# YuxiaWu/RAG4DyG

Measured on AMD Instinct MI355X. Metric: query-seqs/sec encode+top-k over full pool, higher is better.
Workload: dtype f32 (f16x2 operands: two fp16 terms, three products, f32 accumulate)

## Files before the change

include/r4d.h:

```cpp
#ifndef R4D_H
#define R4D_H

#include <stddef.h>
#include <stdint.h>

#ifdef __cplusplus
extern "C" {
#endif

#define R4D_OK 0
#define R4D_ERR_INVALID (-1)
#define R4D_ERR_HIP (-2)
#define R4D_ERR_WORKSPACE (-3)

#define R4D_ABI_VERSION 6

int r4d_abi_version(void);
int r4d_build_flags(void);
const char* r4d_last_error(void);

typedef struct r4d_gpt2_config {
    int32_t n_layer;
    int32_t n_head;
    int32_t n_embd;
// ... 80 lines not shown

int r4d_lm_logits_f32(const float* hidden_d, const float* wte_d, int32_t M, int32_t V, int32_t d,
                      float* logits_d, void* stream);

int r4d_set_attention_fused(int32_t mode);

int r4d_set_attention_h2(int32_t on);
int r4d_set_attention_kblk(int32_t on);
int r4d_pack_kblk_words(const uint32_t* qkv_words_d, int64_t rows, int32_t n_head, int32_t d, uint32_t* kblk_d, void* stream);
int r4d_attention_h2_kblk_f32(const uint32_t* qkv_words_d, const uint32_t* kblk_d, int32_t B, int32_t T, int32_t n_head, int32_t d,
                              float* a_d, void* stream);
int r4d_pack_h2_words_f32(const float* x_d, int64_t n, uint32_t* words_d, void* stream);
int r4d_attention_h2_f32(const uint32_t* qkv_words_d, int32_t B, int32_t T, int32_t n_head, int32_t d, float* a_d, void* stream);

int r4d_set_gemm_h2p(int32_t on);
int r4d_layernorm_lines_f32(const float* x_d, const float* w_d, const float* b_d, int32_t rows, int32_t d, float eps,
                            uint16_t* y_lines_d, void* stream);
int r4d_split2_lines_f16(const float* x_d, int64_t rows, int32_t K, uint16_t* lines_d, void* stream);
int r4d_conv1d_h2p_f32(const uint16_t* x_lines_d, const uint16_t* planes_d, const float* bias_d, const float* residual_d, int32_t M,
                       int32_t K, int32_t N, int32_t epilogue, int32_t out_lines, void* y_d, void* stream);

#define R4D_RANGE_NONFINITE_HIDDEN 1u
#define R4D_RANGE_BAD_NORM 2u
#define R4D_RANGE_BAD_LABEL 4u
int r4d_set_range_flag(uint32_t* flag_d);

int r4d_layernorm_f32(const float* x_d, const float* w_d, const float* b_d, int32_t rows, int32_t d,
                      float eps, float* y_d, void* stream);
int r4d_conv1d_f32(const float* x_d, const float* w_d, const float* w_t_d ,
                   const float* bias_d, const float* residual_d,
// ... 150 lines not shown
```

rag4dyg_amd/_lib.py:

```python
import ctypes
import os
from ctypes import POINTER, Structure, c_char_p, c_double, c_float, c_int32, c_int64, c_size_t, c_uint32, c_uint64, c_void_p

PKG = os.path.dirname(os.path.abspath(__file__))
LIB_PATH = os.environ.get("R4D_LIB_PATH") or os.path.join(PKG, "librag4dyg_hip.so")

R4D_ABI_VERSION = 6
HEAD_GRAD_UNTIED, HEAD_GRAD_TIED, HEAD_GRAD_NONE = 0, 1, 2


class R4DError(RuntimeError):
    pass


class GPT2ConfigC(Structure):
    _fields_ = [("n_layer", c_int32), ("n_head", c_int32), ("n_embd", c_int32), ("vocab", c_int32),
                ("n_positions", c_int32), ("ln_eps", c_float)]


class GPT2LayerC(Structure):
    _fields_ = [(n, c_void_p) for n in ("ln_1_w", "ln_1_b", "c_attn_w", "c_attn_b", "attn_proj_w", "attn_proj_b",
                                         "ln_2_w", "ln_2_b", "c_fc_w", "c_fc_b", "mlp_proj_w", "mlp_proj_b",
                                         "c_attn_wT", "attn_proj_wT", "c_fc_wT", "mlp_proj_wT",
                                         "c_attn_w3", "attn_proj_w3", "c_fc_w3", "mlp_proj_w3",
# ... 38 lines not shown
    "r4d_gpt2_workspace_bytes": (c_size_t, [POINTER(GPT2ConfigC), c_int32, c_int32]),
    "r4d_gpt2_encode_f32": (c_int32, [POINTER(GPT2ConfigC), POINTER(GPT2WeightsC), _P, _P, c_int32, c_int32,
                                      _P, _P, _P, _P, _P, c_size_t, _P]),
    "r4d_gpt2_groups_workspace_bytes": (c_size_t, [POINTER(GPT2ConfigC), c_int32, POINTER(c_int32), POINTER(c_int32)]),
    "r4d_gpt2_encode_groups_f32": (c_int32, [POINTER(GPT2ConfigC), POINTER(GPT2WeightsC), c_int32, POINTER(_P),
                                             POINTER(c_int32), POINTER(c_int32), _P, _P, c_size_t, _P]),
    "r4d_gpt2_encode_groups_ex_f32": (c_int32, [POINTER(GPT2ConfigC), POINTER(GPT2WeightsC), c_int32, POINTER(_P), POINTER(_P),
                                                POINTER(c_int32), POINTER(c_int32), _P, _P, _P, _P, c_size_t, _P]),
    "r4d_set_attention_fused": (c_int32, [c_int32]),
    "r4d_set_attention_h2": (c_int32, [c_int32]),
    "r4d_set_attention_kblk": (c_int32, [c_int32]),
    "r4d_pack_kblk_words": (c_int32, [_P, c_int64, c_int32, c_int32, _P, _P]),
    "r4d_attention_h2_kblk_f32": (c_int32, [_P, _P, c_int32, c_int32, c_int32, c_int32, _P, _P]),
    "r4d_set_range_flag": (c_int32, [_P]),
    "r4d_set_gemm_h2p": (c_int32, [c_int32]),
    "r4d_layernorm_lines_f32": (c_int32, [_P, _P, _P, c_int32, c_int32, c_float, _P, _P]),
    "r4d_split2_lines_f16": (c_int32, [_P, c_int64, c_int32, _P, _P]),
    "r4d_conv1d_h2p_f32": (c_int32, [_P, _P, _P, _P, c_int32, c_int32, c_int32, c_int32, c_int32, _P, _P]),
    "r4d_pack_h2_words_f32": (c_int32, [_P, c_int64, _P, _P]),
    "r4d_attention_h2_f32": (c_int32, [_P, c_int32, c_int32, c_int32, c_int32, _P, _P]),
    "r4d_gpt2_decode_workspace_bytes": (c_size_t, [POINTER(GPT2ConfigC), c_int32]),
    "r4d_gpt2_decode_step_f32": (c_int32, [POINTER(GPT2ConfigC), POINTER(GPT2WeightsC), _P, _P, _P, _P, c_int32, c_int32,
                                           _P, _P, c_size_t, _P]),
    "r4d_gpt2_greedy_workspace_bytes": (c_size_t, [POINTER(GPT2ConfigC), c_int32]),
    "r4d_gpt2_greedy_step_f32": (c_int32, [POINTER(GPT2ConfigC), POINTER(GPT2WeightsC), POINTER(GreedyStateC), _P, c_int32,
                                           c_int32, _P, c_size_t, _P]),
    "r4d_gpt2_greedy_graph_create": (c_int32, [POINTER(GPT2ConfigC), POINTER(GPT2WeightsC), POINTER(GreedyStateC), _P,
                                               c_int32, c_int32, _P, c_size_t, POINTER(_P)]),
    "r4d_decode_graph_launch": (c_int32, [_P, c_int32, _P]),
    "r4d_decode_graph_destroy": (None, [_P]),
# ... 105 lines not shown
```

rag4dyg_amd/csrc/common.h:

```cpp
#pragma once
#include <hip/hip_runtime.h>
#include <stdint.h>
#include <stdio.h>
#include <stdarg.h>
#include "../../include/r4d.h"

namespace r4d {

void set_error(const char* fmt, ...);
int dbgflag_kc(); int dbgflag_att(); int dbgflag_sk(); int dbgflag_jac(); int dbgflag_scan(); int dbgflag_s3(); int dbgflag_h2();

#define R4D_REQUIRE(cond, ...)                     \
    do {                                           \
        if (!(cond)) {                             \
            r4d::set_error(__VA_ARGS__);           \
            return R4D_ERR_INVALID;                \
        }                                          \
    } while (0)

#define R4D_HIP(call)                                                                  \
    do {                                                                               \
        hipError_t e_ = (call);                                                        \
        if (e_ != hipSuccess) {                                                        \
            r4d::set_error("%s: %s", #call, hipGetErrorString(e_));                    \
// ... 101 lines not shown
struct S3Args {
    const float* A; const unsigned short* planes; float* C;
    const float* bias; const float* resid;
    int M, N, K, lda, ldc, ldr, epilogue;
    unsigned* kblk; int kb_hd;
};
bool gemm_s3_supported(int M, int K, int N);
int launch_gemm_s3(const S3Args& a, hipStream_t stream);
bool gemm_s3_f32b_supported(int M, int K, int N);
int launch_gemm_s3_f32b(const float* A, const float* B, float* C, int M, int N, int K, int lda, int ldc, int epilogue, hipStream_t stream);
int launch_gemm_s3_scan_order(const float* q_hat, const float* pool_hat, float* scores, int Q, int N, int d, int ng, hipStream_t stream);
bool gemm_h2_supported(int M, int K, int N);
int launch_gemm_h2(const S3Args& a, hipStream_t stream);
int launch_split2_planes(const float* w, int N, int K, long long ld_k, long long ld_n, unsigned short* planes, hipStream_t s);
extern int g_gemm_h2p;
bool gemm_h2p_supported(int M, int K, int N);
int launch_gemm_h2p(const S3Args& a, const unsigned short* a_lines, bool out_lines, hipStream_t stream);
int launch_split2_lines(const float* x, long long rows, int K, unsigned short* lines, hipStream_t s);
extern int g_gemm_split3;
int conv1d(const float* x, const float* w, const float* wT, const float* bias, const float* resid, int M, int K, int N,
           int epilogue, float* y, hipStream_t s, float* skinny_scratch = nullptr, bool sk_counters_zeroed = false,
           const unsigned short* w3 = nullptr, const unsigned short* w2h = nullptr);
bool gemm_s3tn_supported(int I, int J, int M, int lda, int ldb);
int gemm_s3tn_slices(int I, int J, int M, int max_slices);
int launch_gemm_s3tn(const float* X, const float* dY, float* out, int I, int J, int M, int lda, int ldb, int S, int* slices_out,
                     hipStream_t stream, float* db_partials = nullptr);
int launch_split3_planes(const float* w, int N, int K, long long ld_k, long long ld_n, unsigned short* planes, hipStream_t s);

struct DropKey { unsigned seed_lo, seed_hi, step_lo, step_hi; };
int launch_dropout(const float* x, const float* resid, long long n, float* out, float p, DropKey key, unsigned site,
// ... 90 lines not shown
```

rag4dyg_amd/csrc/gemm_h2p.hip:

```cpp
#include <stdlib.h>
#include <string.h>
#include "common.h"
#include "h2.h"

namespace r4d {

typedef float f32x16p __attribute__((ext_vector_type(16)));
typedef float f32x2p __attribute__((ext_vector_type(2)));
typedef unsigned int u32x4p __attribute__((ext_vector_type(4)));
typedef _Float16 f16x8p __attribute__((ext_vector_type(8)));

int g_gemm_h2p = 1;

__device__ __forceinline__ f32x2p gelu_new_h2p(f32x2p x) {
    const float k0 = -2.0f * 0.7978845608028654f * 1.4426950408889634f, k1 = 0.044715f * k0;
    const f32x2p a = x * x * k1 + k0;
    const f32x2p w = x * a;
    f32x2p e;
    e.x = __builtin_amdgcn_exp2f(w.x); e.y = __builtin_amdgcn_exp2f(w.y);
    e = e + 1.0f;
    f32x2p r;
    r.x = __builtin_amdgcn_rcpf(e.x); r.y = __builtin_amdgcn_rcpf(e.y);
    return x * r;
}
__device__ __forceinline__ float gelu_new_h2p_1(float x) {
    const float k0 = -2.0f * 0.7978845608028654f * 1.4426950408889634f, k1 = 0.044715f * k0;
    return x * __builtin_amdgcn_rcpf(1.0f + __builtin_amdgcn_exp2f(x * __builtin_fmaf(x * x, k1, k0)));
// ... 19 lines not shown
                 "global_load_lds_dwordx4 %2, %5 offset:1024\n\t"
                 "global_load_lds_dwordx4 %3, %5 offset:2048\n\t"
                 "global_load_lds_dwordx4 %4, %5 offset:3072\n\t"
                 "s_mov_b32 m0, %0"
                 : "=&s"(keep) : "v"(v0), "v"(v1), "v"(v2), "v"(v3), "s"(base), "s"(lds_dst) : "memory");
}
template <int N_> __device__ __forceinline__ void h2p_wait_vm() { asm volatile("s_waitcnt vmcnt(%0)" :: "n"(N_) : "memory"); }

template <int BM, int BN, int EPI, bool OUT_LINES, int WGM = 2, int WGN = 4>
__global__ __launch_bounds__(64 * WGM * WGN, (WGM * WGN) / 4) void gemm_h2p_kernel(const unsigned short* __restrict__ Al, const unsigned short* __restrict__ Bp,
                                                          float* __restrict__ Cg, const float* __restrict__ biasg,
                                                          const float* __restrict__ residg, const H2PShape g) {
    constexpr int NW = WGM * WGN;
    constexpr int WM = BM / WGM, WN = BN / WGN, TM = WM / 32, TN = WN / 32;
    constexpr int STAGE = (BM + BN) * 8;
    constexpr int NBUF = 3;
    constexpr int NGA = BM / 8 / NW, NGB = BN / 8 / NW;
    constexpr int NDMA = NGA + NGB;
    static_assert(BM == 128 && (BN == 256 || BN == 128) && TM >= 1 && TN >= 1 && (NGA == 2 || NGA == 4) && (NGB == 2 || NGB == 4 || NGB == 8), "tile");
    __shared__ u32x4p lds[NBUF * STAGE];

    const int nblk = gridDim.x, xq = nblk >> 3, xr = nblk & 7, xcd = blockIdx.x & 7;
    const int bid = xcd * xq + min(xcd, xr) + (blockIdx.x >> 3);
    constexpr int GROUP_M = 8;
    const int tiles_m = (g.M + BM - 1) / BM, tiles_n = (g.N + BN - 1) / BN;
    const int per_group = GROUP_M * tiles_n;
    const int grp = bid / per_group, first_m = grp * GROUP_M;
    const int gsz = min(tiles_m - first_m, GROUP_M);
    const int tile_m = first_m + (bid % per_group) % gsz, tile_n = (bid % per_group) / gsz;
    const int m0 = tile_m * BM, n0 = tile_n * BN;
    const int nkt = g.K / 32;

    const int tid = threadIdx.x, lane = tid & 63, wid = tid >> 6;
    const int wm = wid / WGN, wn = wid % WGN;
    const int li = lane & 31, lh = lane >> 5;

    unsigned va[NGA], vb[NGB];
    const int lrow = lane >> 3, lslot = lane & 7;
#pragma unroll
    for (int i = 0; i < NGA; ++i) {
        const int r = (wid * NGA + i) * 8 + lrow;
        va[i] = (unsigned)min(m0 + r, g.M - 1) * (unsigned)(g.K * 4) + 16u * (unsigned)(lslot ^ ((r >> 1) & 7)) + 3072u - 1024u * (i & 3);
    }
#pragma unroll
    for (int i = 0; i < NGB; ++i) {
        const int r = (wid * NGB + i) * 8 + lrow;
        vb[i] = (unsigned)min(n0 + r, g.N - 1) * (unsigned)(g.K * 4) + 16u * (unsigned)(lslot ^ ((r >> 1) & 7)) + 3072u - 1024u * (i & 3);
    }
    const unsigned lds0 = __builtin_amdgcn_readfirstlane((unsigned)(size_t)lds);
    const unsigned wid_s = __builtin_amdgcn_readfirstlane((unsigned)wid);
    const unsigned dst_a = lds0 + (wid_s * NGA) * 1024u, dst_b = lds0 + ((unsigned)(BM / 8) + wid_s * NGB) * 1024u;
    const char* abase = reinterpret_cast<const char*>(Al) - 3072;
    const char* bbase = reinterpret_cast<const char*>(Bp) - 3072;
#define H2P_ISSUE(KT, STG)                                                                         \
    {                                                                                              \
        const unsigned so_ = (unsigned)(STG) * (unsigned)(STAGE * 16);                             \
        if constexpr (NGA == 4) h2p_dma4(abase + (size_t)(KT) * 128, va[0], va[1], va[2], va[3], dst_a + so_); \
        else h2p_dma2(abase + (size_t)(KT) * 128, va[0], va[1], dst_a + so_);                      \
        if constexpr (NGB == 8) {                                                                  \
            h2p_dma4(bbase + (size_t)(KT) * 128, vb[0], vb[1], vb[2], vb[3], dst_b + so_);          \
            h2p_dma4(bbase + (size_t)(KT) * 128, vb[4], vb[5], vb[6], vb[7], dst_b + so_ + 4096u);   \
        } else if constexpr (NGB == 4) h2p_dma4(bbase + (size_t)(KT) * 128, vb[0], vb[1], vb[2], vb[3], dst_b + so_); \
        else h2p_dma2(bbase + (size_t)(KT) * 128, vb[0], vb[1], dst_b + so_);                       \
    }

    const int fsw = (li >> 1) & 7;
    int f_off[2][2];
#pragma unroll
    for (int s_ = 0; s_ < 2; ++s_)
#pragma unroll
        for (int p = 0; p < 2; ++p) f_off[s_][p] = li * 8 + ((4 * p + 2 * s_ + lh) ^ fsw);
    const int fa_base = wm * WM * 8, fb_base = BM * 8 + wn * WN * 8;

    f32x16p acc0[TM][TN], acc1[TM][TN];
#pragma unroll
    for (int i = 0; i < TM; ++i)
#pragma unroll
        for (int j = 0; j < TN; ++j)
#pragma unroll
            for (int r = 0; r < 16; ++r) { acc0[i][j][r] = 0.f; acc1[i][j][r] = 0.f; }

#define H2P_MFMA(ACC, A_, B_, I_, J_) \
    ACC[I_][J_] = __builtin_amdgcn_mfma_f32_32x32x16_f16(__builtin_bit_cast(f16x8p, A_), __builtin_bit_cast(f16x8p, B_), ACC[I_][J_], 0, 0, 0);
    u32x4p fa[2][TM][2], fb[2][TN][2];
#define H2P_FRAGS(SET, STG, S)                                                                     \
    {                                                                                              \
        const u32x4p* st_ = lds + (STG) * STAGE;                                                   \
                                        \
        _Pragma("unroll") for (int i = 0; i < TM; ++i) fa[SET][i][1] = st_[fa_base + i * 256 + f_off[S][1]]; \
        _Pragma("unroll") for (int j = 0; j < TN; ++j) fb[SET][j][0] = st_[fb_base + j * 256 + f_off[S][0]]; \
        _Pragma("unroll") for (int i = 0; i < TM; ++i) fa[SET][i][0] = st_[fa_base + i * 256 + f_off[S][0]]; \
        _Pragma("unroll") for (int j = 0; j < TN; ++j) fb[SET][j][1] = st_[fb_base + j * 256 + f_off[S][1]]; \
    }
#define H2P_MFMAS(SET)                                                                             \
    {                                                                                              \
        _Pragma("unroll") for (int i = 0; i < TM; ++i) _Pragma("unroll") for (int j = 0; j < TN; ++j) H2P_MFMA(acc1, fa[SET][i][1], fb[SET][j][0], i, j) \
        _Pragma("unroll") for (int i = 0; i < TM; ++i) _Pragma("unroll") for (int j = 0; j < TN; ++j) H2P_MFMA(acc0, fa[SET][i][0], fb[SET][j][0], i, j) \
        _Pragma("unroll") for (int i = 0; i < TM; ++i) _Pragma("unroll") for (int j = 0; j < TN; ++j) H2P_MFMA(acc1, fa[SET][i][0], fb[SET][j][1], i, j) \
    }

    H2P_ISSUE(0, 0)
    if (nkt > 1) { H2P_ISSUE(1, 1) h2p_wait_vm<NDMA>(); } else { h2p_wait_vm<0>(); }
    __syncthreads();
    H2P_FRAGS(0, 0, 0)

    constexpr int NMF = 3 * TM * TN, NFR = 2 * (TM + TN);
    static_assert(NMF >= NFR, "interleave");
#define H2P_ITER(CUR, NXT, WR)                                                                     \
    {                                                                                              \
        __builtin_amdgcn_sched_barrier(0);                                                         \
        const bool more_ = kt + 2 < nkt;                                                           \
        if (more_) H2P_ISSUE(kt + 2, WR)                                                           \
        H2P_FRAGS(1, CUR, 1)                                                                       \
        H2P_MFMAS(0)                                                                               \
        _Pragma("unroll") for (int m_ = 0; m_ < NMF; ++m_) {                                       \
            __builtin_amdgcn_sched_group_barrier(0x008, 1, 0);                                     \
            if (m_ < NFR) __builtin_amdgcn_sched_group_barrier(0x100, 1, 0);                       \
        }                                                                                          \
        __builtin_amdgcn_sched_barrier(0);                                                         \
        if (more_) h2p_wait_vm<NDMA>(); else h2p_wait_vm<0>();                                     \
        asm volatile("s_waitcnt lgkmcnt(0)\n\ts_barrier" ::: "memory");                            \
        H2P_FRAGS(0, NXT, 0)                                                                       \
        H2P_MFMAS(1)                                                                               \
        _Pragma("unroll") for (int m_ = 0; m_ < NMF; ++m_) {                                       \
            __builtin_amdgcn_sched_group_barrier(0x008, 1, 0);                                     \
            if (m_ < NFR) __builtin_amdgcn_sched_group_barrier(0x100, 1, 0);                       \
        }                                                                                          \
        __builtin_amdgcn_sched_barrier(0);                                                         \
    }
    int kt = 0;
    for (; kt + 2 < nkt; kt += 3) {
        H2P_ITER(0, 1, 2)
        { ++kt; H2P_ITER(1, 2, 0) }
        { ++kt; H2P_ITER(2, 0, 1) }
        kt -= 2;
    }
    if (kt < nkt) {
        H2P_ITER(0, 1, 2)
        if (kt + 1 < nkt) { ++kt; H2P_ITER(1, 2, 0) }
    }
#undef H2P_ITER
#undef H2P_FRAGS
#undef H2P_MFMAS
#undef H2P_MFMA
#undef H2P_ISSUE

    constexpr float UNS = H2_A_UNSCALE;
    float* __restrict__ C = Cg;
    const bool interior = (m0 + BM <= g.M) & (n0 + BN <= g.N);
    if constexpr (OUT_LINES) {
        static_assert(EPI == EPI_GELU, "line output: the c_fc epilogue only");
        unsigned char* __restrict__ L = reinterpret_cast<unsigned char*>(Cg);
        const long long row_bytes = (long long)g.N * 4;
        const bool odd = li & 1;
#pragma unroll
        for (int j = 0; j < TN; ++j) {
            const int colb = n0 + wn * WN + j * 32;
            const bool col_ok = colb + li < g.N;
            const float bias = (biasg && col_ok) ? biasg[colb + li] : 0.f;
#pragma unroll
            for (int i = 0; i < TM; ++i) {
#pragma unroll
                for (int r2 = 0; r2 < 16; r2 += 2) {
                    f32x2p v2 = {__builtin_fmaf(acc1[i][j][r2], H2_LO_UNSCALE, acc0[i][j][r2]) * UNS + bias,
                                 __builtin_fmaf(acc1[i][j][r2 + 1], H2_LO_UNSCALE, acc0[i][j][r2 + 1]) * UNS + bias};
                    v2 = gelu_new_h2p(v2);
                    const float vx = v2.x, vy = v2.y;
                    const float send = odd ? vx : vy;
                    const float recv = __builtin_bit_cast(float, __builtin_amdgcn_mov_dpp(__builtin_bit_cast(int, send), 0xB1, 0xF, 0xF, true));
                    const float c0 = odd ? recv : vx, c1 = odd ? vy : recv;
                    unsigned h, l;
                    split2_pair<true>(c0, c1, h, l);
                    const int r = r2 + (odd ? 1 : 0);
                    const int row = m0 + wm * WM + i * 32 + (r & 3) + 8 * (r >> 2) + 4 * lh;
                    if (interior || (row < g.M && col_ok)) {
                        unsigned* dst = reinterpret_cast<unsigned*>(L + (long long)row * row_bytes + (long long)(colb >> 5) * 128 + (li >> 1) * 4);
                        dst[0] = h;
                        dst[16] = l;
                    }
                }
            }
        }
        return;
    } else {
        if (interior) {
            const int lane_c = ((wm * WM + 4 * lh) * g.ldc + wn * WN + li) * 4;
            const int lane_r = ((wm * WM + 4 * lh) * g.ldr + wn * WN + li) * 4;
            const __amdgpu_buffer_rsrc_t c_rsrc = __builtin_amdgcn_make_buffer_rsrc(
                C + (long long)m0 * g.ldc + n0, 0, ((BM - 1) * g.ldc + BN) * 4, 0x00020000);
            const __amdgpu_buffer_rsrc_t r_rsrc = __builtin_amdgcn_make_buffer_rsrc(
                const_cast<float*>(EPI == EPI_RESIDUAL ? residg + (long long)m0 * g.ldr + n0 : Cg), 0,
                EPI == EPI_RESIDUAL ? ((BM - 1) * g.ldr + BN) * 4 : 0, 0x00020000);
            const int kd = g.N / 3;
            const __amdgpu_buffer_rsrc_t kb_rsrc = __builtin_amdgcn_make_buffer_rsrc(
                (EPI == EPI_H2WORDS && g.kb_hd) ? g.kblk : reinterpret_cast<unsigned*>(Cg), 0,
                (EPI == EPI_H2WORDS && g.kb_hd) ? ((g.M + 31) / 32) * (kd * 128) : 0, 0x00020000);
            const int lane_kb = (li >> 3) * 1024 + ((li >> 2) & 1) * 512 + ((li & 3) + 4 * lh) * 16;
#pragma unroll
            for (int j = 0; j < TN; ++j) {
                const float bias = biasg ? biasg[n0 + wn * WN + j * 32 + li] : 0.f;
                const int colb = n0 + wn * WN + j * 32;
                const bool to_kb = EPI == EPI_H2WORDS && g.kb_hd && colb >= kd && colb < 2 * kd;
                const int kb_chunk = to_kb ? ((colb - kd) / g.kb_hd) * (g.kb_hd / 8) + ((colb - kd) % g.kb_hd) / 8 : 0;
#pragma unroll
                for (int i = 0; i < TM; ++i) {
                    const int kb_soff = (((m0 + wm * WM + i * 32) >> 5) * (kd / 8) + kb_chunk) * 1024;
                    float res[16];
                    if (EPI == EPI_RESIDUAL) {
#pragma unroll
                        for (int r = 0; r < 16; ++r)
                            res[r] = __builtin_bit_cast(float, __builtin_amdgcn_raw_buffer_load_b32(
                                r_rsrc, lane_r, ((i * 32 + (r & 3) + 8 * (r >> 2)) * g.ldr + j * 32) * 4, 0));
                    }
                    unsigned o[16];
#pragma unroll
                    for (int r2 = 0; r2 < 16; r2 += 2) {
                        f32x2p v2 = {__builtin_fmaf(acc1[i][j][r2], H2_LO_UNSCALE, acc0[i][j][r2]) * UNS + bias,
                                     __builtin_fmaf(acc1[i][j][r2 + 1], H2_LO_UNSCALE, acc0[i][j][r2 + 1]) * UNS + bias};
                        if (EPI == EPI_GELU) v2 = gelu_new_h2p(v2);
                        else if (EPI == EPI_RESIDUAL) { v2.x += res[r2]; v2.y += res[r2 + 1]; }
                        const float vx = v2.x, vy = v2.y;
                        o[r2] = __builtin_bit_cast(unsigned int, vx); o[r2 + 1] = __builtin_bit_cast(unsigned int, vy);
                        if (EPI == EPI_H2WORDS) h2_words<true>(v2.x, v2.y, o[r2], o[r2 + 1]);
                    }
                    if (EPI == EPI_H2WORDS && to_kb) {
                        const bool o1 = li & 1, o2 = li & 2;
#pragma unroll
                        for (int a4 = 0; a4 < 16; a4 += 4) {
                            unsigned x0 = o[a4], x1 = o[a4 + 1], x2 = o[a4 + 2], x3 = o[a4 + 3];
                            {
                                const unsigned s01 = o1 ? x0 : x1, s23 = o1 ? x2 : x3;
                                const unsigned r01 = (unsigned)__builtin_amdgcn_mov_dpp((int)s01, 0xB1, 0xF, 0xF, true);
                                const unsigned r23 = (unsigned)__builtin_amdgcn_mov_dpp((int)s23, 0xB1, 0xF, 0xF, true);
                                if (o1) { x0 = r01; x2 = r23; } else { x1 = r01; x3 = r23; }
                            }
                            {
                                const unsigned s02 = o2 ? x0 : x2, s13 = o2 ? x1 : x3;
                                const unsigned r02 = (unsigned)__builtin_amdgcn_mov_dpp((int)s02, 0x4E, 0xF, 0xF, true);
                                const unsigned r13 = (unsigned)__builtin_amdgcn_mov_dpp((int)s13, 0x4E, 0xF, 0xF, true);
                                if (o2) { x0 = r02; x1 = r13; } else { x2 = r02; x3 = r13; }
                            }
                            const u32x4p slot = {x0, x1, x2, x3};
                            __builtin_amdgcn_raw_buffer_store_b128(slot, kb_rsrc, lane_kb, kb_soff + 2 * a4 * 16, 0);
                        }
                    } else {
#pragma unroll
                        for (int r = 0; r < 16; ++r)
                            __builtin_amdgcn_raw_buffer_store_b32(o[r], c_rsrc, lane_c, ((i * 32 + (r & 3) + 8 * (r >> 2)) * g.ldc + j * 32) * 4, 0);
                    }
                }
            }
            return;
        }
#pragma unroll
        for (int j = 0; j < TN; ++j) {
            const int col = n0 + wn * WN + j * 32 + li;
            const bool col_ok = col < g.N;
            const int colc = min(col, g.N - 1);
            const float bias = biasg ? biasg[colc] : 0.f;
#pragma unroll
            for (int i = 0; i < TM; ++i) {
#pragma unroll
                for (int r = 0; r < 16; ++r) {
                    const int row = m0 + wm * WM + i * 32 + (r & 3) + 8 * (r >> 2) + 4 * lh;
                    float v = __builtin_fmaf(acc1[i][j][r], H2_LO_UNSCALE, acc0[i][j][r]) * UNS + bias;
                    if (EPI == EPI_GELU) v = gelu_new_h2p_1(v);
                    else if (EPI == EPI_RESIDUAL) v += residg[(long long)min(row, g.M - 1) * g.ldr + colc];
                    else if (EPI == EPI_H2WORDS) { unsigned w0, w1; h2_words<true>(v, 0.f, w0, w1); v = __builtin_bit_cast(float, w0); }
                    if (EPI == EPI_H2WORDS && g.kb_hd && col >= g.N / 3 && col < 2 * (g.N / 3)) {
                        const int kd = g.N / 3, e = (col - kd) % g.kb_hd, chunk = ((col - kd) / g.kb_hd) * (g.kb_hd / 8) + (e >> 3);
                        if (row < g.M)
                            g.kblk[((long long)(row >> 5) * (kd / 8) + chunk) * 256 + (((e >> 2) & 1) * 32 + (row & 31)) * 4 + (e & 3)] =
                                __builtin_bit_cast(unsigned, v);
                        continue;
                    }
                    if (row < g.M && col_ok) C[(long long)row * g.ldc + col] = v;
                }
            }
        }
    }
}

__global__ __launch_bounds__(256) void split2_lines_kernel(const float* __restrict__ x, long long n4, uint2* __restrict__ lines, int K) {
    const long long i = (long long)blockIdx.x * 256 + threadIdx.x;
    if (i >= n4) return;
    const float4 v = reinterpret_cast<const float4*>(x)[i];
    unsigned h0, l0, h1, l1;
    split2_pair<true>(v.x, v.y, h0, l0);
    split2_pair<true>(v.z, v.w, h1, l1);
    const long long e = i * 4, row = e / K;
    const int k = (int)(e - row * K);
    unsigned char* dst = reinterpret_cast<unsigned char*>(lines) + row * (long long)K * 4 + (k >> 5) * 128 + (k & 31) * 2;
    *reinterpret_cast<uint2*>(dst) = make_uint2(h0, h1);
    *reinterpret_cast<uint2*>(dst + 64) = make_uint2(l0, l1);
}

bool gemm_h2p_supported(int M, int K, int N) {
    return g_gemm_h2p != 0 && gemm_h2_supported(M, K, N) && (long long)M * K * 4 + 4096 < (1ll << 32) && (long long)N * K * 4 + 4096 < (1ll << 32);
}

template <int BN>
static int launch_h2p(const S3Args& a, const unsigned short* a_lines, bool out_lines, int cls, hipStream_t stream) {
    const int tiles = cdiv(a.M, 128) * cdiv(a.N, BN);
    ProfScope prof(cls, 2.0 * (double)a.M * a.N * a.K, stream);
    H2PShape sh;
    sh.M = a.M; sh.N = a.N; sh.K = a.K; sh.ldc = a.ldc; sh.ldr = a.ldr;
    sh.kblk = a.kblk; sh.kb_hd = a.kblk ? a.kb_hd : 0;
#define H2P_LAUNCH_(E, OL) hipLaunchKernelGGL((gemm_h2p_kernel<128, BN, E, OL>), dim3(tiles), dim3(512), 0, stream, a_lines, a.planes, a.C, a.bias, a.resid, sh)
    if (out_lines) {
        if (a.epilogue != EPI_GELU) { set_error("gemm_h2p: line output exists for the GELU epilogue only"); return R4D_ERR_INVALID; }
        H2P_LAUNCH_(EPI_GELU, true);
    } else {
        switch (a.epilogue) {
            case EPI_NONE: H2P_LAUNCH_(EPI_NONE, false); break;
            case EPI_GELU: H2P_LAUNCH_(EPI_GELU, false); break;
            case EPI_RESIDUAL: H2P_LAUNCH_(EPI_RESIDUAL, false); break;
            case EPI_H2WORDS: H2P_LAUNCH_(EPI_H2WORDS, false); break;
            default: set_error("gemm_h2p: epilogue %d has no instantiation", a.epilogue); return R4D_ERR_INVALID;
        }
    }
#undef H2P_LAUNCH_
    R4D_CHECK_LAUNCH("gemm_h2p");
    return R4D_OK;
// ... 24 lines not shown
    return R4D_OK;
}

}

using namespace r4d;

extern "C" {

int r4d_set_gemm_h2p(int32_t on) {
    const int prev = g_gemm_h2p;
    g_gemm_h2p = on != 0;
    return prev;
}

int r4d_split2_lines_f16(const float* x_d, int64_t rows, int32_t K, uint16_t* lines_d, void* stream) {
    return launch_split2_lines(x_d, rows, K, lines_d, (hipStream_t)stream);
}

int r4d_conv1d_h2p_f32(const uint16_t* x_lines_d, const uint16_t* planes_d, const float* bias_d, const float* residual_d, int32_t M,
                       int32_t K, int32_t N, int32_t epilogue, int32_t out_lines, void* y_d, void* stream) {
    R4D_REQUIRE(epilogue >= 0 && epilogue <= 2, "conv1d_h2p: epilogue %d not in {0,1,2}", epilogue);
    S3Args a;
    memset(&a, 0, sizeof(a));
    a.planes = planes_d; a.C = (float*)y_d; a.bias = bias_d; a.resid = residual_d;
    a.M = M; a.N = N; a.K = K; a.lda = K; a.ldc = N; a.ldr = N; a.epilogue = epilogue;
    return launch_gemm_h2p(a, x_lines_d, out_lines != 0, (hipStream_t)stream);
}

}
// ... 1 lines not shown
```

rag4dyg_amd/ops.py:

```python
import torch

from . import _lib
from ._lib import check


def _stream():
    return torch.cuda.current_stream().cuda_stream


def _dev(t, dtype, name):
    if not isinstance(t, torch.Tensor) or not t.is_cuda:
        raise _lib.R4DError(f"{name}: expected a tensor on the GPU (no CPU fallback in rag4dyg_amd)")
    if t.dtype != dtype:
        raise _lib.R4DError(f"{name}: expected dtype {dtype}, got {t.dtype}")
    if not t.is_contiguous():
        raise _lib.R4DError(f"{name}: tensor must be contiguous")
    return t.data_ptr()


_WS = {}


def workspace(nbytes, device, tag="default"):
    key = (str(device), tag)
# ... 79 lines not shown
    amax = float(w.detach().abs().max())
    if not (amax < H2_MAX_WEIGHT):
        return None
    if K % 32:
        raise ValueError(f"split2_planes: K = {K} is not a multiple of 32")
    planes = torch.empty(N, K // 32, 2, 32, dtype=torch.int16, device=w.device)
    check(_lib.load().r4d_split2_planes_f16(_dev(w, torch.float32, "w"), K, N, int(bool(transposed)), planes.data_ptr(),
                                            _stream()), "split2_planes")
    return planes


def set_gemm_h2p(on):
    return bool(_lib.load().r4d_set_gemm_h2p(1 if on else 0))


def split2_lines(x):
    K = x.shape[-1]
    rows = x.numel() // K
    out = torch.empty(rows, K // 32, 2, 32, dtype=torch.int16, device=x.device)
    check(_lib.load().r4d_split2_lines_f16(_dev(x, torch.float32, "x"), rows, K, out.data_ptr(), _stream()), "split2_lines")
    return out


def layernorm_lines(x, w, b, eps=1e-5):
    d = x.shape[-1]
    rows = x.numel() // d
    y = torch.empty(rows, d // 32, 2, 32, dtype=torch.int16, device=x.device)
    check(_lib.load().r4d_layernorm_lines_f32(_dev(x, torch.float32, "x"), _dev(w, torch.float32, "w"), _dev(b, torch.float32, "b"),
                                              rows, d, eps, y.data_ptr(), _stream()), "layernorm_lines")
    return y
# ... 267 lines not shown
```

Measured before the change: 39980.

## Make h2p GEMM kernel persistent with next-tile prefetch overlapping epilogue

Converts the split-fp16 MFMA GEMM into a persistent kernel. The grid is capped at the CU count rounded down to a multiple of 8, and each block loops over tiles in strides of gridDim. Before running the epilogue of the current tile, it issues the first two DMA stages of the next tile, so global loads overlap with output stores and launch/tail overhead is reduced. This adds loop-carried register pressure and a one-block-per-CU occupancy assumption, and the new tile-mapping scheme could cause load imbalance when the tile count is not a multiple of the grid.

```diff
diff --git a/include/r4d.h b/include/r4d.h
--- a/include/r4d.h
+++ b/include/r4d.h
@@ -118,6 +118,7 @@
 int r4d_attention_h2_f32(const uint32_t* qkv_words_d, int32_t B, int32_t T, int32_t n_head, int32_t d, float* a_d, void* stream);
 
 int r4d_set_gemm_h2p(int32_t on);
+int r4d_set_gemm_h2p_persistent(int32_t on);
 int r4d_layernorm_lines_f32(const float* x_d, const float* w_d, const float* b_d, int32_t rows, int32_t d, float eps,
                             uint16_t* y_lines_d, void* stream);
 int r4d_split2_lines_f16(const float* x_d, int64_t rows, int32_t K, uint16_t* lines_d, void* stream);
diff --git a/rag4dyg_amd/_lib.py b/rag4dyg_amd/_lib.py
--- a/rag4dyg_amd/_lib.py
+++ b/rag4dyg_amd/_lib.py
@@ -76,6 +76,7 @@
     "r4d_attention_h2_kblk_f32": (c_int32, [_P, _P, c_int32, c_int32, c_int32, c_int32, _P, _P]),
     "r4d_set_range_flag": (c_int32, [_P]),
     "r4d_set_gemm_h2p": (c_int32, [c_int32]),
+    "r4d_set_gemm_h2p_persistent": (c_int32, [c_int32]),
     "r4d_layernorm_lines_f32": (c_int32, [_P, _P, _P, c_int32, c_int32, c_float, _P, _P]),
     "r4d_split2_lines_f16": (c_int32, [_P, c_int64, c_int32, _P, _P]),
     "r4d_conv1d_h2p_f32": (c_int32, [_P, _P, _P, _P, c_int32, c_int32, c_int32, c_int32, c_int32, _P, _P]),
diff --git a/rag4dyg_amd/csrc/common.h b/rag4dyg_amd/csrc/common.h
--- a/rag4dyg_amd/csrc/common.h
+++ b/rag4dyg_amd/csrc/common.h
@@ -139,6 +139,7 @@
 int launch_gemm_h2(const S3Args& a, hipStream_t stream);
 int launch_split2_planes(const float* w, int N, int K, long long ld_k, long long ld_n, unsigned short* planes, hipStream_t s);
 extern int g_gemm_h2p;
+extern int g_gemm_h2p_persistent;
 bool gemm_h2p_supported(int M, int K, int N);
 int launch_gemm_h2p(const S3Args& a, const unsigned short* a_lines, bool out_lines, hipStream_t stream);
 int launch_split2_lines(const float* x, long long rows, int K, unsigned short* lines, hipStream_t s);
diff --git a/rag4dyg_amd/csrc/gemm_h2p.hip b/rag4dyg_amd/csrc/gemm_h2p.hip
--- a/rag4dyg_amd/csrc/gemm_h2p.hip
+++ b/rag4dyg_amd/csrc/gemm_h2p.hip
@@ -11,6 +11,7 @@
 typedef _Float16 f16x8p __attribute__((ext_vector_type(8)));
 
 int g_gemm_h2p = 1;
+int g_gemm_h2p_persistent = 1;
 
 __device__ __forceinline__ f32x2p gelu_new_h2p(f32x2p x) {
     const float k0 = -2.0f * 0.7978845608028654f * 1.4426950408889634f, k1 = 0.044715f * k0;
@@ -60,22 +61,27 @@
     constexpr int NW = WGM * WGN;
     constexpr int WM = BM / WGM, WN = BN / WGN, TM = WM / 32, TN = WN / 32;
     constexpr int STAGE = (BM + BN) * 8;
+    constexpr int NGA = BM / 8 / NW, NGB = BN / 8 / NW;
     constexpr int NBUF = 3;
-    constexpr int NGA = BM / 8 / NW, NGB = BN / 8 / NW;
     constexpr int NDMA = NGA + NGB;
     static_assert(BM == 128 && (BN == 256 || BN == 128) && TM >= 1 && TN >= 1 && (NGA == 2 || NGA == 4) && (NGB == 2 || NGB == 4 || NGB == 8), "tile");
     __shared__ u32x4p lds[NBUF * STAGE];
 
-    const int nblk = gridDim.x, xq = nblk >> 3, xr = nblk & 7, xcd = blockIdx.x & 7;
-    const int bid = xcd * xq + min(xcd, xr) + (blockIdx.x >> 3);
     constexpr int GROUP_M = 8;
     const int tiles_m = (g.M + BM - 1) / BM, tiles_n = (g.N + BN - 1) / BN;
+    const int ntiles = tiles_m * tiles_n, xq = ntiles >> 3, xr = ntiles & 7;
     const int per_group = GROUP_M * tiles_n;
-    const int grp = bid / per_group, first_m = grp * GROUP_M;
-    const int gsz = min(tiles_m - first_m, GROUP_M);
-    const int tile_m = first_m + (bid % per_group) % gsz, tile_n = (bid % per_group) / gsz;
-    const int m0 = tile_m * BM, n0 = tile_n * BN;
     const int nkt = g.K / 32;
+#define H2P_TILE(V, M0_, N0_)                                                                      \
+    {                                                                                              \
+        const int xcd_ = (V) & 7, bid_ = xcd_ * xq + min(xcd_, xr) + ((V) >> 3);                   \
+        const int grp_ = bid_ / per_group, first_m_ = grp_ * GROUP_M;                              \
+        const int gsz_ = min(tiles_m - first_m_, GROUP_M);                                         \
+        M0_ = (first_m_ + (bid_ % per_group) % gsz_) * BM;                                         \
+        N0_ = ((bid_ % per_group) / gsz_) * BN;                                                    \
+    }
+    int v = blockIdx.x, m0, n0;
+    H2P_TILE(v, m0, n0)
 
     const int tid = threadIdx.x, lane = tid & 63, wid = tid >> 6;
     const int wm = wid / WGN, wn = wid % WGN;
@@ -83,16 +89,18 @@
 
     unsigned va[NGA], vb[NGB];
     const int lrow = lane >> 3, lslot = lane & 7;
-#pragma unroll
-    for (int i = 0; i < NGA; ++i) {
-        const int r = (wid * NGA + i) * 8 + lrow;
-        va[i] = (unsigned)min(m0 + r, g.M - 1) * (unsigned)(g.K * 4) + 16u * (unsigned)(lslot ^ ((r >> 1) & 7)) + 3072u - 1024u * (i & 3);
-    }
-#pragma unroll
-    for (int i = 0; i < NGB; ++i) {
-        const int r = (wid * NGB + i) * 8 + lrow;
-        vb[i] = (unsigned)min(n0 + r, g.N - 1) * (unsigned)(g.K * 4) + 16u * (unsigned)(lslot ^ ((r >> 1) & 7)) + 3072u - 1024u * (i & 3);
-    }
+#define H2P_LANES(M0_, N0_)                                                                        \
+    {                                                                                              \
+        _Pragma("unroll") for (int i = 0; i < NGA; ++i) {                                          \
+            const int r = (wid * NGA + i) * 8 + lrow;                       \
+            va[i] = (unsigned)min((M0_) + r, g.M - 1) * (unsigned)(g.K * 4) + 16u * (unsigned)(lslot ^ ((r >> 1) & 7)) + 3072u - 1024u * (i & 3); \
+        }                                                                                          \
+        _Pragma("unroll") for (int i = 0; i < NGB; ++i) {                                          \
+            const int r = (wid * NGB + i) * 8 + lrow;                       \
+            vb[i] = (unsigned)min((N0_) + r, g.N - 1) * (unsigned)(g.K * 4) + 16u * (unsigned)(lslot ^ ((r >> 1) & 7)) + 3072u - 1024u * (i & 3); \
+        }                                                                                          \
+    }
+    H2P_LANES(m0, n0)
     const unsigned lds0 = __builtin_amdgcn_readfirstlane((unsigned)(size_t)lds);
     const unsigned wid_s = __builtin_amdgcn_readfirstlane((unsigned)wid);
     const unsigned dst_a = lds0 + (wid_s * NGA) * 1024u, dst_b = lds0 + ((unsigned)(BM / 8) + wid_s * NGB) * 1024u;
@@ -119,13 +127,6 @@
     const int fa_base = wm * WM * 8, fb_base = BM * 8 + wn * WN * 8;
 
     f32x16p acc0[TM][TN], acc1[TM][TN];
-#pragma unroll
-    for (int i = 0; i < TM; ++i)
-#pragma unroll
-        for (int j = 0; j < TN; ++j)
-#pragma unroll
-            for (int r = 0; r < 16; ++r) { acc0[i][j][r] = 0.f; acc1[i][j][r] = 0.f; }
-
 #define H2P_MFMA(ACC, A_, B_, I_, J_) \
     ACC[I_][J_] = __builtin_amdgcn_mfma_f32_32x32x16_f16(__builtin_bit_cast(f16x8p, A_), __builtin_bit_cast(f16x8p, B_), ACC[I_][J_], 0, 0, 0);
     u32x4p fa[2][TM][2], fb[2][TN][2];
@@ -145,10 +146,6 @@
         _Pragma("unroll") for (int i = 0; i < TM; ++i) _Pragma("unroll") for (int j = 0; j < TN; ++j) H2P_MFMA(acc1, fa[SET][i][0], fb[SET][j][1], i, j) \
     }
 
-    H2P_ISSUE(0, 0)
-    if (nkt > 1) { H2P_ISSUE(1, 1) h2p_wait_vm<NDMA>(); } else { h2p_wait_vm<0>(); }
-    __syncthreads();
-    H2P_FRAGS(0, 0, 0)
 
     constexpr int NMF = 3 * TM * TN, NFR = 2 * (TM + TN);
     static_assert(NMF >= NFR, "interleave");
@@ -174,157 +171,191 @@
         }                                                                                          \
         __builtin_amdgcn_sched_barrier(0);                                                         \
     }
-    int kt = 0;
-    for (; kt + 2 < nkt; kt += 3) {
-        H2P_ITER(0, 1, 2)
-        { ++kt; H2P_ITER(1, 2, 0) }
-        { ++kt; H2P_ITER(2, 0, 1) }
-        kt -= 2;
-    }
-    if (kt < nkt) {
-        H2P_ITER(0, 1, 2)
-        if (kt + 1 < nkt) { ++kt; H2P_ITER(1, 2, 0) }
+
+    H2P_ISSUE(0, 0)
+    if (nkt > 1) H2P_ISSUE(1, 1)
+    for (bool first = true;; first = false) {
+        const int vn = v + (int)gridDim.x;
+        const bool has_next = vn < ntiles;
+        int m0n = 0, n0n = 0;
+        if (has_next) H2P_TILE(vn, m0n, n0n)
+#pragma unroll
+        for (int i = 0; i < TM; ++i)
+#pragma unroll
+            for (int j = 0; j < TN; ++j)
+#pragma unroll
+                for (int r = 0; r < 16; ++r) { acc0[i][j][r] = 0.f; acc1[i][j][r] = 0.f; }
+
+        if (first && nkt > 1) h2p_wait_vm<NDMA>(); else h2p_wait_vm<0>();
+        asm volatile("s_barrier" ::: "memory");
+        H2P_FRAGS(0, 0, 0)
+
+        int kt = 0;
+        for (; kt + 2 < nkt; kt += 3) {
+            H2P_ITER(0, 1, 2)
+            { ++kt; H2P_ITER(1, 2, 0) }
+            { ++kt; H2P_ITER(2, 0, 1) }
+            kt -= 2;
+        }
+        if (kt < nkt) {
+            H2P_ITER(0, 1, 2)
+            if (kt + 1 < nkt) { ++kt; H2P_ITER(1, 2, 0) }
+        }
+
+        if (has_next) {
+            asm volatile("s_waitcnt lgkmcnt(0)\n\ts_barrier" ::: "memory");
+            H2P_LANES(m0n, n0n)
+            H2P_ISSUE(0, 0)
+            if (nkt > 1) H2P_ISSUE(1, 1)
+        }
+
+        constexpr float UNS = H2_A_UNSCALE;
+        float* __restrict__ C = Cg;
+        const bool interior = (m0 + BM <= g.M) & (n0 + BN <= g.N);
+        if constexpr (OUT_LINES) {
+            static_assert(EPI == EPI_GELU, "line output: the c_fc epilogue only");
+            unsigned char* __restrict__ L = reinterpret_cast<unsigned char*>(Cg);
+            const long long row_bytes = (long long)g.N * 4;
+            const bool odd = li & 1;
+#pragma unroll
+            for (int j = 0; j < TN; ++j) {
+                const int colb = n0 + wn * WN + j * 32;
+                const bool col_ok = colb + li < g.N;
+                const float bias = (biasg && col_ok) ? biasg[colb + li] : 0.f;
+#pragma unroll
+                for (int i = 0; i < TM; ++i) {
+#pragma unroll
+                    for (int r2 = 0; r2 < 16; r2 += 2) {
+                        f32x2p v2 = {__builtin_fmaf(acc1[i][j][r2], H2_LO_UNSCALE, acc0[i][j][r2]) * UNS + bias,
+                                     __builtin_fmaf(acc1[i][j][r2 + 1], H2_LO_UNSCALE, acc0[i][j][r2 + 1]) * UNS + bias};
+                        v2 = gelu_new_h2p(v2);
+                        const float vx = v2.x, vy = v2.y;
+                        const float send = odd ? vx : vy;
+                        const float recv = __builtin_bit_cast(float, __builtin_amdgcn_mov_dpp(__builtin_bit_cast(int, send), 0xB1, 0xF, 0xF, true));
+                        const float c0 = odd ? recv : vx, c1 = odd ? vy : recv;
+                        unsigned h, l;
+                        split2_pair<true>(c0, c1, h, l);
+                        const int r = r2 + (odd ? 1 : 0);
+                        const int row = m0 + wm * WM + i * 32 + (r & 3) + 8 * (r >> 2) + 4 * lh;
+                        if (interior || (row < g.M && col_ok)) {
+                            unsigned* dst = reinterpret_cast<unsigned*>(L + (long long)row * row_bytes + (long long)(colb >> 5) * 128 + (li >> 1) * 4);
+                            dst[0] = h;
+                            dst[16] = l;
+                        }
+                    }
+                }
+            }
+        } else {
+            if (interior) {
+                int ldc = g.ldc, ldr = g.ldr;
+                asm volatile("" : "+s"(ldc), "+s"(ldr));
+                const int lane_c = ((wm * WM + 4 * lh) * ldc + wn * WN + li) * 4;
+                const int lane_r = ((wm * WM + 4 * lh) * ldr + wn * WN + li) * 4;
+                const __amdgpu_buffer_rsrc_t c_rsrc = __builtin_amdgcn_make_buffer_rsrc(
+                    C + (long long)m0 * ldc + n0, 0, ((BM - 1) * ldc + BN) * 4, 0x00020000);
+                const __amdgpu_buffer_rsrc_t r_rsrc = __builtin_amdgcn_make_buffer_rsrc(
+                    const_cast<float*>(EPI == EPI_RESIDUAL ? residg + (long long)m0 * ldr + n0 : Cg), 0,
+                    EPI == EPI_RESIDUAL ? ((BM - 1) * ldr + BN) * 4 : 0, 0x00020000);
+                const int kd = g.N / 3;
+                const __amdgpu_buffer_rsrc_t kb_rsrc = __builtin_amdgcn_make_buffer_rsrc(
+                    (EPI == EPI_H2WORDS && g.kb_hd) ? g.kblk : reinterpret_cast<unsigned*>(Cg), 0,
+                    (EPI == EPI_H2WORDS && g.kb_hd) ? ((g.M + 31) / 32) * (kd * 128) : 0, 0x00020000);
+                const int lane_kb = (li >> 3) * 1024 + ((li >> 2) & 1) * 512 + ((li & 3) + 4 * lh) * 16;
+#pragma unroll
+                for (int j = 0; j < TN; ++j) {
+                    const float bias = biasg ? biasg[n0 + wn * WN + j * 32 + li] : 0.f;
+                    const int colb = n0 + wn * WN + j * 32;
+                    const bool to_kb = EPI == EPI_H2WORDS && g.kb_hd && colb >= kd && colb < 2 * kd;
+                    const int kb_chunk = to_kb ? ((colb - kd) / g.kb_hd) * (g.kb_hd / 8) + ((colb - kd) % g.kb_hd) / 8 : 0;
+#pragma unroll
+                    for (int i = 0; i < TM; ++i) {
+                        const int kb_soff = (((m0 + wm * WM + i * 32) >> 5) * (kd / 8) + kb_chunk) * 1024;
+                        float res[16];
+                        if (EPI == EPI_RESIDUAL) {
+#pragma unroll
+                            for (int r = 0; r < 16; ++r)
+                                res[r] = __builtin_bit_cast(float, __builtin_amdgcn_raw_buffer_load_b32(
+                                    r_rsrc, lane_r, ((i * 32 + (r & 3) + 8 * (r >> 2)) * ldr + j * 32) * 4, 0));
+                        }
+                        unsigned o[16];
+#pragma unroll
+                        for (int r2 = 0; r2 < 16; r2 += 2) {
+                            f32x2p v2 = {__builtin_fmaf(acc1[i][j][r2], H2_LO_UNSCALE, acc0[i][j][r2]) * UNS + bias,
+                                         __builtin_fmaf(acc1[i][j][r2 + 1], H2_LO_UNSCALE, acc0[i][j][r2 + 1]) * UNS + bias};
+                            if (EPI == EPI_GELU) v2 = gelu_new_h2p(v2);
+                            else if (EPI == EPI_RESIDUAL) { v2.x += res[r2]; v2.y += res[r2 + 1]; }
+                            const float vx = v2.x, vy = v2.y;
+                            o[r2] = __builtin_bit_cast(unsigned int, vx); o[r2 + 1] = __builtin_bit_cast(unsigned int, vy);
+                            if (EPI == EPI_H2WORDS) h2_words<true>(v2.x, v2.y, o[r2], o[r2 + 1]);
+                        }
+                        if (EPI == EPI_H2WORDS && to_kb) {
+                            const bool o1 = li & 1, o2 = li & 2;
+#pragma unroll
+                            for (int a4 = 0; a4 < 16; a4 += 4) {
+                                unsigned x0 = o[a4], x1 = o[a4 + 1], x2 = o[a4 + 2], x3 = o[a4 + 3];
+                                {
+                                    const unsigned s01 = o1 ? x0 : x1, s23 = o1 ? x2 : x3;
+                                    const unsigned r01 = (unsigned)__builtin_amdgcn_mov_dpp((int)s01, 0xB1, 0xF, 0xF, true);
+                                    const unsigned r23 = (unsigned)__builtin_amdgcn_mov_dpp((int)s23, 0xB1, 0xF, 0xF, true);
+                                    if (o1) { x0 = r01; x2 = r23; } else { x1 = r01; x3 = r23; }
+                                }
+                                {
+                                    const unsigned s02 = o2 ? x0 : x2, s13 = o2 ? x1 : x3;
+                                    const unsigned r02 = (unsigned)__builtin_amdgcn_mov_dpp((int)s02, 0x4E, 0xF, 0xF, true);
+                                    const unsigned r13 = (unsigned)__builtin_amdgcn_mov_dpp((int)s13, 0x4E, 0xF, 0xF, true);
+                                    if (o2) { x0 = r02; x1 = r13; } else { x2 = r02; x3 = r13; }
+                                }
+                                const u32x4p slot = {x0, x1, x2, x3};
+                                __builtin_amdgcn_raw_buffer_store_b128(slot, kb_rsrc, lane_kb, kb_soff + 2 * a4 * 16, 0);
+                            }
+                        } else {
+#pragma unroll
+                            for (int r = 0; r < 16; ++r)
+                                __builtin_amdgcn_raw_buffer_store_b32(o[r], c_rsrc, lane_c, ((i * 32 + (r & 3) + 8 * (r >> 2)) * ldc + j * 32) * 4, 0);
+                        }
+                    }
+                }
+            } else {
+#pragma unroll
+                for (int j = 0; j < TN; ++j) {
+                    const int col = n0 + wn * WN + j * 32 + li;
+                    const bool col_ok = col < g.N;
+                    const int colc = min(col, g.N - 1);
+                    const float bias = biasg ? biasg[colc] : 0.f;
+#pragma unroll
+                    for (int i = 0; i < TM; ++i) {
+                        int Me = g.M;
+                        asm volatile("" : "+s"(Me));
+#pragma unroll
+                        for (int r = 0; r < 16; ++r) {
+                            const int row = m0 + wm * WM + i * 32 + (r & 3) + 8 * (r >> 2) + 4 * lh;
+                            float v = __builtin_fmaf(acc1[i][j][r], H2_LO_UNSCALE, acc0[i][j][r]) * UNS + bias;
+                            if (EPI == EPI_GELU) v = gelu_new_h2p_1(v);
+                            else if (EPI == EPI_RESIDUAL) v += residg[(long long)min(row, Me - 1) * g.ldr + colc];
+                            else if (EPI == EPI_H2WORDS) { unsigned w0, w1; h2_words<true>(v, 0.f, w0, w1); v = __builtin_bit_cast(float, w0); }
+                            if (EPI == EPI_H2WORDS && g.kb_hd && col >= g.N / 3 && col < 2 * (g.N / 3)) {
+                                const int kd = g.N / 3, e = (col - kd) % g.kb_hd, chunk = ((col - kd) / g.kb_hd) * (g.kb_hd / 8) + (e >> 3);
+                                if (row < Me)
+                                    g.kblk[((long long)(row >> 5) * (kd / 8) + chunk) * 256 + (((e >> 2) & 1) * 32 + (row & 31)) * 4 + (e & 3)] =
+                                        __builtin_bit_cast(unsigned, v);
+                                continue;
+                            }
+                            if (row < Me && col_ok) C[(long long)row * g.ldc + col] = v;
+                        }
+                    }
+                }
+            }
+        }
+        if (!has_next) break;
+        v = vn; m0 = m0n; n0 = n0n;
     }
 #undef H2P_ITER
 #undef H2P_FRAGS
 #undef H2P_MFMAS
 #undef H2P_MFMA
 #undef H2P_ISSUE
-
-    constexpr float UNS = H2_A_UNSCALE;
-    float* __restrict__ C = Cg;
-    const bool interior = (m0 + BM <= g.M) & (n0 + BN <= g.N);
-    if constexpr (OUT_LINES) {
-        static_assert(EPI == EPI_GELU, "line output: the c_fc epilogue only");
-        unsigned char* __restrict__ L = reinterpret_cast<unsigned char*>(Cg);
-        const long long row_bytes = (long long)g.N * 4;
-        const bool odd = li & 1;
-#pragma unroll
-        for (int j = 0; j < TN; ++j) {
-            const int colb = n0 + wn * WN + j * 32;
-            const bool col_ok = colb + li < g.N;
-            const float bias = (biasg && col_ok) ? biasg[colb + li] : 0.f;
-#pragma unroll
-            for (int i = 0; i < TM; ++i) {
-#pragma unroll
-                for (int r2 = 0; r2 < 16; r2 += 2) {
-                    f32x2p v2 = {__builtin_fmaf(acc1[i][j][r2], H2_LO_UNSCALE, acc0[i][j][r2]) * UNS + bias,
-                                 __builtin_fmaf(acc1[i][j][r2 + 1], H2_LO_UNSCALE, acc0[i][j][r2 + 1]) * UNS + bias};
-                    v2 = gelu_new_h2p(v2);
-                    const float vx = v2.x, vy = v2.y;
-                    const float send = odd ? vx : vy;
-                    const float recv = __builtin_bit_cast(float, __builtin_amdgcn_mov_dpp(__builtin_bit_cast(int, send), 0xB1, 0xF, 0xF, true));
-                    const float c0 = odd ? recv : vx, c1 = odd ? vy : recv;
-                    unsigned h, l;
-                    split2_pair<true>(c0, c1, h, l);
-                    const int r = r2 + (odd ? 1 : 0);
-                    const int row = m0 + wm * WM + i * 32 + (r & 3) + 8 * (r >> 2) + 4 * lh;
-                    if (interior || (row < g.M && col_ok)) {
-                        unsigned* dst = reinterpret_cast<unsigned*>(L + (long long)row * row_bytes + (long long)(colb >> 5) * 128 + (li >> 1) * 4);
-                        dst[0] = h;
-                        dst[16] = l;
-                    }
-                }
-            }
-        }
-        return;
-    } else {
-        if (interior) {
-            const int lane_c = ((wm * WM + 4 * lh) * g.ldc + wn * WN + li) * 4;
-            const int lane_r = ((wm * WM + 4 * lh) * g.ldr + wn * WN + li) * 4;
-            const __amdgpu_buffer_rsrc_t c_rsrc = __builtin_amdgcn_make_buffer_rsrc(
-                C + (long long)m0 * g.ldc + n0, 0, ((BM - 1) * g.ldc + BN) * 4, 0x00020000);
-            const __amdgpu_buffer_rsrc_t r_rsrc = __builtin_amdgcn_make_buffer_rsrc(
-                const_cast<float*>(EPI == EPI_RESIDUAL ? residg + (long long)m0 * g.ldr + n0 : Cg), 0,
-                EPI == EPI_RESIDUAL ? ((BM - 1) * g.ldr + BN) * 4 : 0, 0x00020000);
-            const int kd = g.N / 3;
-            const __amdgpu_buffer_rsrc_t kb_rsrc = __builtin_amdgcn_make_buffer_rsrc(
-                (EPI == EPI_H2WORDS && g.kb_hd) ? g.kblk : reinterpret_cast<unsigned*>(Cg), 0,
-                (EPI == EPI_H2WORDS && g.kb_hd) ? ((g.M + 31) / 32) * (kd * 128) : 0, 0x00020000);
-            const int lane_kb = (li >> 3) * 1024 + ((li >> 2) & 1) * 512 + ((li & 3) + 4 * lh) * 16;
-#pragma unroll
-            for (int j = 0; j < TN; ++j) {
-                const float bias = biasg ? biasg[n0 + wn * WN + j * 32 + li] : 0.f;
-                const int colb = n0 + wn * WN + j * 32;
-                const bool to_kb = EPI == EPI_H2WORDS && g.kb_hd && colb >= kd && colb < 2 * kd;
-                const int kb_chunk = to_kb ? ((colb - kd) / g.kb_hd) * (g.kb_hd / 8) + ((colb - kd) % g.kb_hd) / 8 : 0;
-#pragma unroll
-                for (int i = 0; i < TM; ++i) {
-                    const int kb_soff = (((m0 + wm * WM + i * 32) >> 5) * (kd / 8) + kb_chunk) * 1024;
-                    float res[16];
-                    if (EPI == EPI_RESIDUAL) {
-#pragma unroll
-                        for (int r = 0; r < 16; ++r)
-                            res[r] = __builtin_bit_cast(float, __builtin_amdgcn_raw_buffer_load_b32(
-                                r_rsrc, lane_r, ((i * 32 + (r & 3) + 8 * (r >> 2)) * g.ldr + j * 32) * 4, 0));
-                    }
-                    unsigned o[16];
-#pragma unroll
-                    for (int r2 = 0; r2 < 16; r2 += 2) {
-                        f32x2p v2 = {__builtin_fmaf(acc1[i][j][r2], H2_LO_UNSCALE, acc0[i][j][r2]) * UNS + bias,
-                                     __builtin_fmaf(acc1[i][j][r2 + 1], H2_LO_UNSCALE, acc0[i][j][r2 + 1]) * UNS + bias};
-                        if (EPI == EPI_GELU) v2 = gelu_new_h2p(v2);
-                        else if (EPI == EPI_RESIDUAL) { v2.x += res[r2]; v2.y += res[r2 + 1]; }
-                        const float vx = v2.x, vy = v2.y;
-                        o[r2] = __builtin_bit_cast(unsigned int, vx); o[r2 + 1] = __builtin_bit_cast(unsigned int, vy);
-                        if (EPI == EPI_H2WORDS) h2_words<true>(v2.x, v2.y, o[r2], o[r2 + 1]);
-                    }
-                    if (EPI == EPI_H2WORDS && to_kb) {
-                        const bool o1 = li & 1, o2 = li & 2;
-#pragma unroll
-                        for (int a4 = 0; a4 < 16; a4 += 4) {
-                            unsigned x0 = o[a4], x1 = o[a4 + 1], x2 = o[a4 + 2], x3 = o[a4 + 3];
-                            {
-                                const unsigned s01 = o1 ? x0 : x1, s23 = o1 ? x2 : x3;
-                                const unsigned r01 = (unsigned)__builtin_amdgcn_mov_dpp((int)s01, 0xB1, 0xF, 0xF, true);
-                                const unsigned r23 = (unsigned)__builtin_amdgcn_mov_dpp((int)s23, 0xB1, 0xF, 0xF, true);
-                                if (o1) { x0 = r01; x2 = r23; } else { x1 = r01; x3 = r23; }
-                            }
-                            {
-                                const unsigned s02 = o2 ? x0 : x2, s13 = o2 ? x1 : x3;
-                                const unsigned r02 = (unsigned)__builtin_amdgcn_mov_dpp((int)s02, 0x4E, 0xF, 0xF, true);
-                                const unsigned r13 = (unsigned)__builtin_amdgcn_mov_dpp((int)s13, 0x4E, 0xF, 0xF, true);
-                                if (o2) { x0 = r02; x1 = r13; } else { x2 = r02; x3 = r13; }
-                            }
-                            const u32x4p slot = {x0, x1, x2, x3};
-                            __builtin_amdgcn_raw_buffer_store_b128(slot, kb_rsrc, lane_kb, kb_soff + 2 * a4 * 16, 0);
-                        }
-                    } else {
-#pragma unroll
-                        for (int r = 0; r < 16; ++r)
-                            __builtin_amdgcn_raw_buffer_store_b32(o[r], c_rsrc, lane_c, ((i * 32 + (r & 3) + 8 * (r >> 2)) * g.ldc + j * 32) * 4, 0);
-                    }
-                }
-            }
-            return;
-        }
-#pragma unroll
-        for (int j = 0; j < TN; ++j) {
-            const int col = n0 + wn * WN + j * 32 + li;
-            const bool col_ok = col < g.N;
-            const int colc = min(col, g.N - 1);
-            const float bias = biasg ? biasg[colc] : 0.f;
-#pragma unroll
-            for (int i = 0; i < TM; ++i) {
-#pragma unroll
-                for (int r = 0; r < 16; ++r) {
-                    const int row = m0 + wm * WM + i * 32 + (r & 3) + 8 * (r >> 2) + 4 * lh;
-                    float v = __builtin_fmaf(acc1[i][j][r], H2_LO_UNSCALE, acc0[i][j][r]) * UNS + bias;
-                    if (EPI == EPI_GELU) v = gelu_new_h2p_1(v);
-                    else if (EPI == EPI_RESIDUAL) v += residg[(long long)min(row, g.M - 1) * g.ldr + colc];
-                    else if (EPI == EPI_H2WORDS) { unsigned w0, w1; h2_words<true>(v, 0.f, w0, w1); v = __builtin_bit_cast(float, w0); }
-                    if (EPI == EPI_H2WORDS && g.kb_hd && col >= g.N / 3 && col < 2 * (g.N / 3)) {
-                        const int kd = g.N / 3, e = (col - kd) % g.kb_hd, chunk = ((col - kd) / g.kb_hd) * (g.kb_hd / 8) + (e >> 3);
-                        if (row < g.M)
-                            g.kblk[((long long)(row >> 5) * (kd / 8) + chunk) * 256 + (((e >> 2) & 1) * 32 + (row & 31)) * 4 + (e & 3)] =
-                                __builtin_bit_cast(unsigned, v);
-                        continue;
-                    }
-                    if (row < g.M && col_ok) C[(long long)row * g.ldc + col] = v;
-                }
-            }
-        }
-    }
+#undef H2P_LANES
+#undef H2P_TILE
 }
 
 __global__ __launch_bounds__(256) void split2_lines_kernel(const float* __restrict__ x, long long n4, uint2* __restrict__ lines, int K) {
@@ -345,14 +376,28 @@
     return g_gemm_h2p != 0 && gemm_h2_supported(M, K, N) && (long long)M * K * 4 + 4096 < (1ll << 32) && (long long)N * K * 4 + 4096 < (1ll << 32);
 }
 
+static int device_cus(int* cus) {
+    static int cached[64];
+    int dev = 0;
+    R4D_HIP(hipGetDevice(&dev));
+    if (dev < 0 || dev >= 64) { set_error("gemm_h2p: device ordinal %d", dev); return R4D_ERR_INVALID; }
+    if (!cached[dev]) R4D_HIP(hipDeviceGetAttribute(&cached[dev], hipDeviceAttributeMultiprocessorCount, dev));
+    *cus = cached[dev];
+    return R4D_OK;
+}
+
 template <int BN>
 static int launch_h2p(const S3Args& a, const unsigned short* a_lines, bool out_lines, int cls, hipStream_t stream) {
     const int tiles = cdiv(a.M, 128) * cdiv(a.N, BN);
+    int cus = 0;
+    if (const int rc = device_cus(&cus)) return rc;
+    const int resident = cus & ~7;
+    const int grid = (g_gemm_h2p_persistent && resident >= 8 && tiles > resident) ? resident : tiles;
     ProfScope prof(cls, 2.0 * (double)a.M * a.N * a.K, stream);
     H2PShape sh;
     sh.M = a.M; sh.N = a.N; sh.K = a.K; sh.ldc = a.ldc; sh.ldr = a.ldr;
     sh.kblk = a.kblk; sh.kb_hd = a.kblk ? a.kb_hd : 0;
-#define H2P_LAUNCH_(E, OL) hipLaunchKernelGGL((gemm_h2p_kernel<128, BN, E, OL>), dim3(tiles), dim3(512), 0, stream, a_lines, a.planes, a.C, a.bias, a.resid, sh)
+#define H2P_LAUNCH_(E, OL) hipLaunchKernelGGL((gemm_h2p_kernel<128, BN, E, OL>), dim3(grid), dim3(512), 0, stream, a_lines, a.planes, a.C, a.bias, a.resid, sh)
     if (out_lines) {
         if (a.epilogue != EPI_GELU) { set_error("gemm_h2p: line output exists for the GELU epilogue only"); return R4D_ERR_INVALID; }
         H2P_LAUNCH_(EPI_GELU, true);
@@ -407,6 +452,12 @@
     return prev;
 }
 
+int r4d_set_gemm_h2p_persistent(int32_t on) {
+    const int prev = g_gemm_h2p_persistent;
+    g_gemm_h2p_persistent = on != 0;
+    return prev;
+}
+
 int r4d_split2_lines_f16(const float* x_d, int64_t rows, int32_t K, uint16_t* lines_d, void* stream) {
     return launch_split2_lines(x_d, rows, K, lines_d, (hipStream_t)stream);
 }
diff --git a/rag4dyg_amd/ops.py b/rag4dyg_amd/ops.py
--- a/rag4dyg_amd/ops.py
+++ b/rag4dyg_amd/ops.py
@@ -117,6 +117,10 @@
     return bool(_lib.load().r4d_set_gemm_h2p(1 if on else 0))
 
 
+def set_gemm_h2p_persistent(on):
+    return bool(_lib.load().r4d_set_gemm_h2p_persistent(1 if on else 0))
+
+
 def split2_lines(x):
     K = x.shape[-1]
     rows = x.numel() // K
```

After: 39560. -1.1%, worse.
